# piyanon108/iGate4xSoftphoneDSP

Hardware: AMD Instinct MI355X
Metric: Msamples/s G.711 decode+RMS, 65536ch@8kHz; %HBM roofline at 1/2/4/8 GPU (higher is better)
Workload: dtype u8

## Files before the change

igate4xsoftphonedsp_amd/csrc/igdsp_capi_ctx.hip:

```cpp
#include "igdsp_ctx.h"

#include <algorithm>
#include <atomic>
#include <cmath>
#include <cstdlib>
#include <cstring>
#include <mutex>
#include <new>
#include <vector>

using namespace igdsp;
using igdsp_rx::kSlot;
using igdsp_rx::kStageDepth;

extern "C" {

int igdsp_abi_version(void) { return IGDSP_ABI_VERSION; }

int igdsp_create(igdsp_ctx **out, int device, uint32_t max_channels)
{
    if (!out || max_channels == 0 || max_channels > (1u << 24)) return IGDSP_EINVAL;
    *out = nullptr;
    int count = 0;
    if (hipGetDeviceCount(&count) != hipSuccess || count <= 0 || device < 0 || device >= count) return IGDSP_ENODEV;
    hipDeviceProp_t prop;
    if (hipGetDeviceProperties(&prop, device) != hipSuccess) return IGDSP_ENODEV;
    if (std::strncmp(prop.gcnArchName, "gfx950", 6) != 0) return IGDSP_ENODEV;
    if (hipSetDevice(device) != hipSuccess) return IGDSP_ENODEV;

    igdsp_ctx *ctx = new (std::nothrow) igdsp_ctx();
    if (!ctx) return IGDSP_ENOMEM;
    ctx->device = device;
    ctx->cus = prop.multiProcessorCount;
    ctx->name = prop.name;
    ctx->max_channels = max_channels;
    ctx->direct = std::vector<std::atomic<uint32_t>>(kDirectCalls);
    for (auto &d : ctx->direct) d.store(kNoChan, std::memory_order_relaxed);
    const size_t max_frames = (size_t)max_channels * kStageDepth;
    ctx->up_bytes = igdsp_rx::upload_layout(max_frames, max_channels).total;
    bool ok = hipStreamCreateWithFlags(&ctx->stream, hipStreamNonBlocking) == hipSuccess;
    ok = ok && hipEventCreateWithFlags(&ctx->flush_done, hipEventDisableTiming) == hipSuccess;
    for (int i = 0; i < igdsp_rx::RingMem::kArrays; ++i)
        ok = ok && hipHostMalloc(ctx->ring.array(i), igdsp_rx::RingMem::bytes(max_channels, i), hipHostMallocDefault) == hipSuccess;
    if (ok) ctx->rx.init(max_channels, ctx->ring);
    ok = ok && hipHostMalloc((void **)&ctx->h_up, ctx->up_bytes, hipHostMallocDefault) == hipSuccess;
    for (uint32_t i = 0; i < 2; ++i) {
        igdsp_rx::Published &pb = ctx->pub.set(i);
        ok = ok && hipHostMalloc((void **)&pb.last, max_channels * sizeof(igdsp_frame_stats), hipHostMallocDefault) == hipSuccess;
        ok = ok && hipHostMalloc((void **)&pb.hold, max_channels * sizeof(igdsp_chan_hold), hipHostMallocDefault) == hipSuccess;
        ok = ok && hipHostMalloc((void **)&pb.probe, max_channels * sizeof(igdsp_chan_probe), hipHostMallocDefault) == hipSuccess;
    }
    ok = ok && hipMalloc((void **)&ctx->d_up, ctx->up_bytes) == hipSuccess;
    ok = ok && hipMalloc((void **)&ctx->d_stats, 2 * max_frames * sizeof(igdsp_frame_stats)) == hipSuccess;
    ok = ok && hipMalloc((void **)&ctx->d_last, max_channels * sizeof(igdsp_frame_stats)) == hipSuccess;
    ok = ok && hipMalloc((void **)&ctx->d_hold, max_channels * sizeof(igdsp_chan_hold)) == hipSuccess;
    ok = ok && hipMalloc((void **)&ctx->d_probe, max_channels * sizeof(igdsp_chan_probe)) == hipSuccess;
    ok = ok && hipMalloc((void **)&ctx->d_queues, kQueueRing * 32u * sizeof(uint32_t)) == hipSuccess;
    ok = ok && hipMemset(ctx->d_queues, 0, kQueueRing * 32u * sizeof(uint32_t)) == hipSuccess;
    ok = ok && hipMemset(ctx->d_last, 0, max_channels * sizeof(igdsp_frame_stats)) == hipSuccess;
    ok = ok && hipMemset(ctx->d_probe, 0, max_channels * sizeof(igdsp_chan_probe)) == hipSuccess;
    if (const char *e = std::getenv("IGDSP_GLOBAL_QUEUE")) ctx->global_queue = std::atoi(e) != 0;
    if (const char *e = std::getenv("IGDSP_IO_SPARE_CHUNKS")) ctx->io_spare_cap = (size_t)std::max(0, std::atoi(e));
    if (!ok) {
        igdsp_destroy(ctx);
        return IGDSP_ENOMEM;
    }
    if (init_device_attributes() != hipSuccess) {
        igdsp_destroy(ctx);
        return IGDSP_EDEVICE;
    }
    bool up = launch_hold_reset(ctx->d_hold, max_channels, nullptr, ctx->stream) == hipSuccess;
    for (uint32_t i = 0; i < 2; ++i) {
        igdsp_rx::Published &pb = ctx->pub.set(i);
        std::memset(pb.last, 0, max_channels * sizeof(igdsp_frame_stats));
        std::memset(pb.probe, 0, max_channels * sizeof(igdsp_chan_probe));
        up = up && hipMemcpyAsync(pb.hold, ctx->d_hold, max_channels * sizeof(igdsp_chan_hold), hipMemcpyDeviceToHost, ctx->stream) == hipSuccess;
    }
    if (!up || hipStreamSynchronize(ctx->stream) != hipSuccess) {
        igdsp_destroy(ctx);
        return IGDSP_EDEVICE;
    }
    ctx->pool = make_pool(max_channels);
    *out = ctx;
    return IGDSP_OK;
}

int igdsp_destroy(igdsp_ctx *ctx)
{
    if (!ctx) return IGDSP_OK;
    ctx->pool.reset();
    if (ctx->device >= 0) (void)hipSetDevice(ctx->device);
    igdsp_tx_drop(ctx);
    igdsp_io_drop_spares(ctx);
    if (ctx->stream) { (void)hipStreamSynchronize(ctx->stream); (void)hipStreamDestroy(ctx->stream); }
    if (ctx->flush_done) (void)hipEventDestroy(ctx->flush_done);
    for (int i = 0; i < igdsp_rx::RingMem::kArrays; ++i) if (*ctx->ring.array(i)) (void)hipHostFree(*ctx->ring.array(i));
    const igdsp_rx::Published &p0 = ctx->pub.set(0), &p1 = ctx->pub.set(1);
    void *hosts[] = {ctx->h_up, p0.last, p0.hold, p0.probe, p1.last, p1.hold, p1.probe};
    for (void *p : hosts) if (p) (void)hipHostFree(p);
    void *devs[] = {ctx->d_up, ctx->d_stats, ctx->d_last, ctx->d_hold, ctx->d_probe, ctx->d_queues, ctx->d_enc_tab[0], ctx->d_enc_tab[1]};
    for (void *p : devs) if (p) (void)hipFree(p);
    delete ctx;
    return IGDSP_OK;
}

const char *igdsp_last_error(const igdsp_ctx *ctx) { return ctx ? ctx->err.c_str() : ""; }

int igdsp_device_info(const igdsp_ctx *ctx, int *device, int *compute_units, char *name, size_t name_len)
{
    if (!ctx) return IGDSP_EINVAL;
    if (device) *device = ctx->device;
    if (compute_units) *compute_units = ctx->cus;
    if (name && name_len) { std::strncpy(name, ctx->name.c_str(), name_len - 1); name[name_len - 1] = 0; }
    return IGDSP_OK;
}

int igdsp_set_variant(igdsp_ctx *ctx, int variant)
{
    if (!ctx || variant < 0 || variant > 4) return IGDSP_EINVAL;
    ctx->variant = variant;
    return IGDSP_OK;
}

int igdsp_map_call(igdsp_ctx *ctx, int32_t call_id, uint32_t channel)
{
    if (!ctx) return IGDSP_EINVAL;
    if (channel >= ctx->max_channels) return IGDSP_ERANGE;
    if (call_id >= 0 && call_id < kDirectCalls) ctx->direct[(size_t)call_id].store(channel, std::memory_order_release);
    else { std::lock_guard<std::mutex> g(ctx->far_mu); ctx->far[call_id] = channel; }
    return IGDSP_OK;
}

int igdsp_unmap_call(igdsp_ctx *ctx, int32_t call_id)
{
    if (!ctx) return IGDSP_EINVAL;
    if (call_id >= 0 && call_id < kDirectCalls) ctx->direct[(size_t)call_id].store(kNoChan, std::memory_order_release);
    else { std::lock_guard<std::mutex> g(ctx->far_mu); ctx->far.erase(call_id); }
    return IGDSP_OK;
}

int igdsp_on_rtp_frame(igdsp_ctx *ctx, int32_t call_id, uint8_t pt, const uint8_t *payload, uint32_t payloadlen)
{
    if (!ctx) return IGDSP_EINVAL;
    if (pt != IGDSP_PT_PCMU && pt != IGDSP_PT_PCMA) return IGDSP_OK;
    if (payloadlen > kSlot || (payloadlen && !payload)) return IGDSP_EINVAL;
// ... 123 lines not shown
    igdsp_frame_stats s;
    uint16_t peak_hold = 0;
    ctx->pub.read([&](const igdsp_rx::Published &p) { s = p.last[channel]; peak_hold = p.hold[channel].peak_hold; });
    out->byte_mean = s.byte_mean;
    out->flags = s.flags;
    out->peak = s.peak;
    out->rms = s.rms;
    out->percent = (int32_t)(float)(((double)s.rms * 100.0) / (double)IGDSP_METER_FULL_SCALE);
    out->peak_hold = peak_hold;
    out->dropped = (uint16_t)std::min<uint32_t>(ctx->rx.frames_dropped(channel), 65535u);
    out->frames = ctx->rx.frames_seen(channel);
    return IGDSP_OK;
}

int igdsp_poll_call(igdsp_ctx *ctx, int32_t call_id, igdsp_level *out)
{
    if (!ctx || !out) return IGDSP_EINVAL;
    const uint32_t ch = lookup(ctx, call_id);
    if (ch == kNoChan) return IGDSP_ENOENT;
    return igdsp_poll(ctx, ch, out);
}

int igdsp_reset_hold(igdsp_ctx *ctx, uint32_t channel)
{
    if (!ctx) return IGDSP_EINVAL;
    if (channel != 0xFFFFFFFFu && channel >= ctx->max_channels) return IGDSP_ERANGE;
    std::lock_guard<std::mutex> g(ctx->flush_mu);
    if (int rc = flush_end_locked(ctx, 1)) return rc;
    HIP_TRY(ctx, hipSetDevice(ctx->device));
    const uint32_t c0 = (channel == 0xFFFFFFFFu) ? 0 : channel;
    const uint32_t cn = (channel == 0xFFFFFFFFu) ? ctx->max_channels : 1;
    HIP_TRY(ctx, launch_hold_reset(ctx->d_hold + c0, cn, nullptr, ctx->stream));
    HIP_TRY(ctx, hipMemcpyAsync(ctx->pub.back().hold + c0, ctx->d_hold + c0, cn * sizeof(igdsp_chan_hold), hipMemcpyDeviceToHost, ctx->stream));
    HIP_TRY(ctx, hipStreamSynchronize(ctx->stream));
    ctx->pub.rewrite_front([&](igdsp_rx::Published &front, const igdsp_rx::Published &back) {
        std::memcpy(front.hold + c0, back.hold + c0, cn * sizeof(igdsp_chan_hold));
    });
    return IGDSP_OK;
}

int igdsp_get_hold(igdsp_ctx *ctx, uint32_t channel, igdsp_chan_hold *out)
{
    if (!ctx || !out) return IGDSP_EINVAL;
    if (channel >= ctx->max_channels) return IGDSP_ERANGE;
    ctx->pub.read([&](const igdsp_rx::Published &p) { *out = p.hold[channel]; });
    return IGDSP_OK;
}

int igdsp_get_probe(igdsp_ctx *ctx, uint32_t channel, igdsp_chan_probe *out)
{
    if (!ctx || !out) return IGDSP_EINVAL;
    if (channel >= ctx->max_channels) return IGDSP_ERANGE;
    ctx->pub.read([&](const igdsp_rx::Published &p) { *out = p.probe[channel]; });
    return IGDSP_OK;
}

int igdsp_dev_alloc(igdsp_ctx *ctx, void **d_ptr, size_t bytes)
{
    if (!ctx || !d_ptr) return IGDSP_EINVAL;
    *d_ptr = nullptr;
    if (bytes == 0) return IGDSP_OK;
    if (hipSetDevice(ctx->device) != hipSuccess) return IGDSP_ENODEV;
    hipError_t e = hipMalloc(d_ptr, bytes);
    return e == hipSuccess ? IGDSP_OK : fail(ctx, IGDSP_ENOMEM, "hipMalloc", e);
}

int igdsp_dev_free(igdsp_ctx *ctx, void *d_ptr)
{
    if (!ctx) return IGDSP_EINVAL;
    if (!d_ptr) return IGDSP_OK;
    HIP_TRY(ctx, hipSetDevice(ctx->device));
    HIP_TRY(ctx, hipFree(d_ptr));
    return IGDSP_OK;
}

int igdsp_dev_alloc_far(igdsp_ctx *ctx, void **d_ptr, size_t bytes, const void *d_in, size_t in_bytes, uint32_t max_tries,
                        size_t spacer_bytes, float *ms_first, float *ms_kept)
{
    if (!ctx || !d_ptr || !d_in || bytes == 0 || in_bytes < 10240u || max_tries == 0) return IGDSP_EINVAL;
    *d_ptr = nullptr;
    if (hipSetDevice(ctx->device) != hipSuccess) return IGDSP_ENODEV;
    if (spacer_bytes == 0) spacer_bytes = (size_t)12 << 30;
    const size_t cand_bytes = std::max(bytes, in_bytes / 10u + 4096u);
    std::vector<void *> spacers;
    void *best = nullptr;
    float t_best = 0.f, t_first = 0.f;
    int rc = IGDSP_OK;
    for (uint32_t k = 0; k < max_tries; ++k) {
        if (k > 0) {
            void *sp = nullptr;
            if (hipMalloc(&sp, spacer_bytes) != hipSuccess) { (void)hipGetLastError(); break; }
            spacers.push_back(sp);
        }
        void *cand = nullptr;
        if (hipMalloc(&cand, cand_bytes) != hipSuccess) { (void)hipGetLastError(); break; }
        float ms = 0.f;
        rc = igdsp_probe_placement(ctx, d_in, in_bytes, cand, 6, &ms, nullptr);
        if (rc != IGDSP_OK) { (void)hipFree(cand); break; }
        if (k == 0) t_first = ms;
        if (best == nullptr || ms < t_best) {
            if (best) (void)hipFree(best);
            best = cand; t_best = ms;
        } else {
            (void)hipFree(cand);
        }
        if (t_best < 0.92f * t_first) break;
    }
    for (void *sp : spacers) (void)hipFree(sp);
    if (rc != IGDSP_OK) { if (best) (void)hipFree(best); return rc; }
    if (!best) return fail(ctx, IGDSP_ENOMEM, "igdsp_dev_alloc_far");
    *d_ptr = best;
    if (ms_first) *ms_first = t_first;
    if (ms_kept) *ms_kept = t_best;
    return IGDSP_OK;
}

int igdsp_copy_h2d(igdsp_ctx *ctx, void *d_dst, const void *h_src, size_t bytes)
{
    if (!ctx || (bytes && (!d_dst || !h_src))) return IGDSP_EINVAL;
    HIP_TRY(ctx, hipSetDevice(ctx->device));
    HIP_TRY(ctx, hipMemcpy(d_dst, h_src, bytes, hipMemcpyHostToDevice));
    return IGDSP_OK;
}

int igdsp_copy_d2h(igdsp_ctx *ctx, void *h_dst, const void *d_src, size_t bytes)
// ... 73 lines not shown
```

igate4xsoftphonedsp_amd/csrc/igdsp_ctx.h:

```cpp
#pragma once
#include "igdsp_args.h"
#include "igdsp_internal.h"
#include "igdsp_rxstage.h"
#include "igdsp_snappool.h"

#include <atomic>
#include <cstdio>
#include <mutex>
#include <string>
#include <unordered_map>
#include <vector>

namespace {
constexpr uint32_t kNoChan = 0xFFFFFFFFu;
constexpr int32_t kDirectCalls = 1 << 16;
}

struct igdsp_ctx {
    int device = -1;
    int cus = 0;
    std::string name;
    uint32_t max_channels = 0;
    hipStream_t stream = nullptr;
    int variant = 0;
    std::string err;

    struct IoRange { const char *base; size_t bytes; };
    std::vector<IoRange> spread_ranges;
    std::vector<hipMemGenericAllocationHandle_t> io_spare[4];
    size_t io_spare_chunk = 0;
    size_t io_spare_cap = 16;
    uint32_t io_epoch = 0;
    std::mutex io_mu;
    bool is_spread(const void *p)
    {
        std::lock_guard<std::mutex> g(io_mu);
        for (const auto &r : spread_ranges) if ((const char *)p >= r.base && (const char *)p < r.base + r.bytes) return true;
        return false;
    }

    std::vector<std::atomic<uint32_t>> direct;
    std::unordered_map<int32_t, uint32_t> far;
    std::mutex far_mu;

    igdsp_rx::RingMem ring;
    igdsp_rx::Stager rx;
    std::atomic<uint32_t> gate_mode{IGDSP_GATE_ALWAYS};

    uint8_t *h_up = nullptr, *d_up = nullptr;
    size_t up_bytes = 0;
    igdsp_frame_stats *d_stats = nullptr;
    igdsp_frame_stats *d_last = nullptr;
    igdsp_chan_hold *d_hold = nullptr;
    igdsp_chan_probe *d_probe = nullptr;
    igdsp_rx::PublishedSet pub;
    hipEvent_t flush_done = nullptr;
    bool flush_open = false;
    uint32_t flush_nch = 0;
    std::mutex flush_mu;

    std::unique_ptr<igdsp::SnapshotPool> pool;

    struct TxSide;
    std::atomic<TxSide *> tx{nullptr};
    std::mutex tx_init_mu;

    uint32_t *d_queues = nullptr;
    uint8_t *d_enc_tab[2] = {nullptr, nullptr};
    std::once_flag enc_once[2];
    hipStream_t queue_owner[64];
    uint32_t queue_launches[64];
    uint32_t queue_used = 0;
    uint32_t queue_hint = 0;
    std::atomic_flag queue_lk = ATOMIC_FLAG_INIT;
    bool global_queue = true;
};
namespace {
constexpr uint32_t kQueueRing = 64;
const hipStream_t kFreeQueue = reinterpret_cast<hipStream_t>(~(uintptr_t)0);
}

void igdsp_io_drop_spares(igdsp_ctx *ctx);
void igdsp_tx_drop(igdsp_ctx *ctx);

static inline uint32_t lookup(igdsp_ctx *ctx, int32_t call_id)
{
    if (call_id >= 0 && call_id < kDirectCalls) return ctx->direct[(size_t)call_id].load(std::memory_order_acquire);
    std::lock_guard<std::mutex> g(ctx->far_mu);
    auto it = ctx->far.find(call_id);
    return it == ctx->far.end() ? kNoChan : it->second;
}

static inline int fail(igdsp_ctx *ctx, int code, const char *what, hipError_t e = hipSuccess)
{
    if (ctx) {
        char buf[256];
        if (e != hipSuccess) std::snprintf(buf, sizeof buf, "%s: %s", what, hipGetErrorString(e));
        else std::snprintf(buf, sizeof buf, "%s", what);
        ctx->err = buf;
    }
    return code;
}

#define HIP_TRY(ctx, call)                                                    \
    do {                                                                      \
        hipError_t e_ = (call);                                               \
        if (e_ != hipSuccess) return fail((ctx), IGDSP_EDEVICE, #call, e_);   \
    } while (0)

static inline int refuse(igdsp_ctx *ctx, const char *entry, const igdsp::args::Verdict &v)
{
    return v.why ? fail(ctx, v.rc, (std::string(entry) + ": " + v.why).c_str()) : v.rc;
}

#define ARGS_TRY(ctx, entry, verdict)                                         \
    do {                                                                      \
        const igdsp::args::Verdict v_ = (verdict);                            \
        if (!v_.run) return refuse((ctx), (entry), v_);                       \
    } while (0)

static inline hipStream_t pick(igdsp_ctx *, void *stream) { return (hipStream_t)stream; }
static inline uint32_t *queue_of(igdsp_ctx *ctx, hipStream_t stream)
{
    if (!ctx->global_queue || !ctx->d_queues || stream == hipStreamPerThread) return nullptr;
    while (ctx->queue_lk.test_and_set(std::memory_order_acquire)) {}
    uint32_t i = ctx->queue_hint;
    if (i >= ctx->queue_used || ctx->queue_owner[i] != stream) {
        uint32_t free_i = kQueueRing;
        for (i = 0; i < ctx->queue_used && ctx->queue_owner[i] != stream; ++i)
            if (ctx->queue_owner[i] == kFreeQueue && free_i == kQueueRing) free_i = i;
        if (i == ctx->queue_used) {
            if (free_i != kQueueRing) i = free_i;
            else if (ctx->queue_used < kQueueRing) ctx->queue_used += 1;
            else i = kQueueRing;
            if (i < kQueueRing) { ctx->queue_owner[i] = stream; ctx->queue_launches[i] = 0; }
// ... 33 lines not shown
```

igate4xsoftphonedsp_amd/csrc/igdsp_io.hip:

```cpp
#include "igdsp_ctx.h"

#include <algorithm>
#include <chrono>
#include <thread>
#include <cmath>
#include <cstdlib>
#include <cstring>
#include <new>

using namespace igdsp;

struct igdsp_io_set {
    struct Map { void *va = nullptr; size_t bytes = 0; std::vector<hipMemGenericAllocationHandle_t> handles; std::vector<uint8_t> cls; };
    uint32_t epoch = 0;
    std::vector<Map> maps;
    std::vector<void *> plain;
    size_t chunk = 0;
    int device = 0;
};

namespace {

constexpr size_t kSrcChunks = 10;

// ... 83 lines not shown
            chunks[idx[k]].in_src = true;
            if (hipMemSetAccess((char *)T.va + k * chunk, chunk, &acc, 1) != hipSuccess) { (void)hipGetLastError(); return false; }
        }
        *which = sources.size() - 1;
        return true;
    }
    void drop_source(size_t which)
    {
        Source &S = sources[which];
        for (size_t k = 0; k < S.idx.size(); ++k) { (void)hipMemUnmap((char *)S.va + k * chunk, chunk); chunks[S.idx[k]].in_src = false; }
        S.idx.clear();
    }
    void cleanup()
    {
        for (size_t i = 0; i < chunks.size(); ++i) unmap_scratch(i);
        for (size_t w = 0; w < sources.size(); ++w) drop_source(w);
        sources.clear();
        for (auto &c : chunks) if (!c.used) (void)hipMemRelease(c.h);
        chunks.clear();
        if (ea) (void)hipEventDestroy(ea);
        if (eb) (void)hipEventDestroy(eb);
        ea = eb = nullptr; cand_va = nullptr;
        (void)hipGetLastError();
    }
};

bool map_chunks(igdsp_io_set::Map &m, size_t chunk, const std::vector<hipMemGenericAllocationHandle_t> &hs, size_t first_slot,
                const hipMemAccessDesc &acc)
{
    for (size_t i = 0; i < hs.size(); ++i) {
        char *at = (char *)m.va + (first_slot + i) * chunk;
        if (hipMemMap(at, chunk, 0, hs[i], 0) != hipSuccess) return false;
        if (hipMemSetAccess(at, chunk, &acc, 1) != hipSuccess) return false;
    }
    return true;
}

struct IoKnobs {
    bool plain = false, frac_set = false, no_spread = false, settle = true, debug = false;
    int align_mib = -1; double limit_frac = 0.0;
    size_t stride = 16;
    IoKnobs()
    {
        if (const char *e = std::getenv("IGDSP_IO_PLAIN")) plain = std::atoi(e) != 0;
        if (const char *e = std::getenv("IGDSP_IO_ALIGN_MIB")) align_mib = std::max(0, std::atoi(e));
        if (const char *e = std::getenv("IGDSP_IO_LIMIT_FRAC")) { frac_set = true; limit_frac = std::atof(e); }
        if (const char *e = std::getenv("IGDSP_IO_STRIDE")) stride = std::max(1, std::atoi(e));
        no_spread = std::getenv("IGDSP_IO_NO_SPREAD") != nullptr;
        if (const char *e = std::getenv("IGDSP_IO_SETTLE")) settle = std::atoi(e) != 0;
        debug = std::getenv("IGDSP_IO_DEBUG") != nullptr;
    }
};
size_t probe_bytes(size_t chunk) { return kSrcChunks * (chunk - 4096) / 10240 * 10240; }
struct Layout {
    std::vector<size_t> nch;
    std::vector<uint32_t> order;
    size_t in_chunks = 0, in_bytes = 0, rec_chunks = 0, bulk_chunks = 0;
    int in0 = -1, out0 = -1;
};
struct Pools {
    std::vector<size_t> a, b, c;
    float fast = 0.f, slow = 0.f, thrB = 0.f, thrC = 0.f;
    bool split = false;
    const std::vector<size_t> &pool(int q) const { return q == 0 ? a : (q == 1 ? b : c); }
    int label(int q) const { return q == 0 ? 0 : (q == 2 ? 3 : (split ? 2 : 1)); }
};
struct Search {
    Explorer &X; const Layout &L; const size_t stride; igdsp_io_report &R;
    Pools P;
    bool ok = true;
    static constexpr float kBimodal = 1.08f, kPure = 1.125f, kNear = 1.035f;
    size_t srcA = 0, srcB = 0, nB = 0, nC = 0;
    float tmin = 1e30f, tmax = 0.f, tbmin = 1e30f, tbmax = 0.f;
    float cB = 0.f, cC = 0.f, thrB = 0.f, thrC = 0.f;
    std::vector<size_t> surveyed; std::vector<char> taken;
    bool timeA(size_t idx)
    {
        Chunk &c = X.chunks[idx];
        if (c.tA >= 0.f || c.in_src) return true;
        if (!X.probe(idx, X.sources[srcA], &c.tA, "A")) return ok = false;
        return true;
    }
    bool fast_A(size_t idx) { return !X.chunks[idx].in_src && timeA(idx) && X.chunks[idx].tA < P.fast; }
    bool timeB(size_t idx)
    {
        Chunk &c = X.chunks[idx];
        if (c.in_src || !ok) return false;
        if (c.tB < 0.f) {
            if (!X.probe(idx, X.sources[srcB], &c.tB, "B")) return ok = false;
            tbmin = std::min(tbmin, c.tB); tbmax = std::max(tbmax, c.tB);
        }
        return true;
    }
    bool is_C(size_t idx) { return fast_A(idx) && timeB(idx) && X.chunks[idx].tB < thrC; }
    bool is_B(size_t idx) { return fast_A(idx) && timeB(idx) && X.chunks[idx].tB > thrB; }
    void survey(bool rescan)
    {
        tmin = 1e30f; tmax = 0.f;
        std::vector<size_t> todo = rescan ? surveyed : std::vector<size_t>();
        surveyed.clear();
        size_t next = 0, seen = 0;
        for (;;) {
            const size_t idx = seen < todo.size() ? todo[seen] : next;
            if (seen >= todo.size() && !X.ensure(idx)) break;
            next = std::max(next, idx) + stride;
            ++seen;
// ... 275 lines not shown
            labels.push_back((uint8_t)P.label(q));
            hs.push_back(c.h);
        }
    };
    for (size_t j = 0; j < L.order.size() && ok; ++j) {
        const uint32_t i = L.order[j];
        hs.clear(); labels.clear();
        if (bufs[i].role == IGDSP_IO_INPUT) pull(0, L.nch[i]);
        else {
            const size_t h2 = (bufs[i].role == IGDSP_IO_BULK && spread) ? L.nch[i] / 2 : 0;
            pull(1, L.nch[i] - h2);
            if (hs.size() == L.nch[i] - h2) pull(2, h2);
        }
        all = all && hs.size() == L.nch[i];
        ok = map_chunks(set->maps[i], set->chunk, hs, 0, X.acc);
        set->maps[i].handles = hs; set->maps[i].cls = labels;
    }
    R.placed = (ok && all) ? 1u : 0u; R.bulk_spread = (ok && all && spread && L.bulk_chunks > 0) ? 1u : 0u;
    if (X.debug && ok) {
        std::fprintf(stderr, "[igdsp_io] pools: A %zu B %zu C %zu chunks; A:", P.a.size(), P.b.size(), P.c.size());
        for (size_t k = 0; k < P.a.size() && k < 12; ++k) std::fprintf(stderr, " %zu", P.a[k]);
        std::fprintf(stderr, "  B:");
        for (size_t k = 0; k < P.b.size() && k < 12; ++k) std::fprintf(stderr, " %zu(%.4f)", P.b[k], X.chunks[P.b[k]].tA);
        std::fprintf(stderr, "\n");
        debug_check(X, bufs, n_bufs, L, set, false);
    }
    return ok;
}
void keep_spares(igdsp_ctx *ctx, Explorer &X, const Pools &P)
{
    for (int q = 0; q < 3; ++q)
        for (size_t k : P.pool(q)) if (!X.chunks[k].used) X.chunks[k].cls = P.label(q);
    for (auto &c : X.chunks) {
        if (c.used || c.in_src || c.cls >= 0 || c.tA < 0.f) continue;
        if (c.tA > P.slow) c.cls = 0;
        else if (c.tA < P.fast) c.cls = !P.split ? 1 : (c.tB > P.thrB ? 2 : ((c.tB >= 0.f && c.tB < P.thrC) ? 3 : -1));
    }
    std::lock_guard<std::mutex> g(ctx->io_mu);
    for (auto &c : X.chunks)
        if (!c.used && !c.in_src && c.cls >= 0 && ctx->io_spare[c.cls].size() < ctx->io_spare_cap) { ctx->io_spare[c.cls].push_back(c.h); c.used = true; }
}
bool map_fresh(igdsp_io_set::Map &m, size_t nch, size_t chunk, const hipMemAllocationProp &prop, const hipMemAccessDesc &acc)
{
    const size_t have = m.handles.size();
    std::vector<hipMemGenericAllocationHandle_t> hs;
    bool ok = true;
    hipMemGenericAllocationHandle_t h;
    for (size_t k = have; k < nch && ok; ++k) if ((ok = hipMemCreate(&h, chunk, &prop, 0) == hipSuccess)) hs.push_back(h);
    ok = ok && map_chunks(m, chunk, hs, have, acc);
    m.handles.insert(m.handles.end(), hs.begin(), hs.end());
    m.cls.resize(m.handles.size(), 255);
    return ok;
}
float settle_ref(Explorer &X, const Layout &L, const igdsp_io_set *set, size_t *n)
{
    if (L.in0 < 0 || L.out0 < 0) return 0.f;
    *n = std::min(X.probe_n, std::min(L.nch[L.in0] * set->chunk, 10 * (L.nch[L.out0] * set->chunk - 4096)) / 10240 * 10240);
    const size_t keep = X.probe_n; X.probe_n = *n;
    float t = 0.f, t_ref = 0.f;
    const void *rd = set->maps[L.in0].va; void *wr = set->maps[L.out0].va;
    if (*n >= ((size_t)256 << 20) && X.time_pair(rd, wr, &t) && X.time_pair(rd, wr, &t)) t_ref = t;
    X.probe_n = keep;
    return t_ref;
}
float settle(igdsp_ctx *ctx, const Layout &L, const igdsp_io_set *set, size_t n, float t_ref, size_t released_chunks, bool debug)
{
    Explorer Y;
    const auto w0 = std::chrono::steady_clock::now();
    if (Y.open(ctx, n)) {
        const float min_wait = std::min(6000.f, (float)((double)released_chunks * (double)set->chunk / 25e9 * 1e3));
        int quiet = 0;
        for (;;) {
            float t = 0.f; if (!Y.time_pair(set->maps[L.in0].va, set->maps[L.out0].va, &t)) break;
            quiet = t <= 1.012f * t_ref ? quiet + 1 : 0;
            const float waited = std::chrono::duration<float, std::milli>(std::chrono::steady_clock::now() - w0).count();
            if (debug) std::fprintf(stderr, "[igdsp_io] settle: %.4f ms against %.4f before the release (%.0f of >= %.0f ms)\n", t, t_ref, waited, min_wait);
            if ((quiet >= 2 && waited >= min_wait) || waited > 8000.f) break;
            std::this_thread::sleep_for(std::chrono::milliseconds(50));
        }
    }
    const float ms = std::chrono::duration<float, std::milli>(std::chrono::steady_clock::now() - w0).count();
    Y.cleanup();
    return ms;
}
int place(igdsp_ctx *ctx, igdsp_io_buf *bufs, uint32_t n_bufs, size_t explore_limit_bytes, const IoKnobs &kn, igdsp_io_set *set,
          Explorer &X, igdsp_io_report &R)
{
    int vmm = 0;
    if (hipDeviceGetAttribute(&vmm, hipDeviceAttributeVirtualMemoryManagementSupported, ctx->device) != hipSuccess) { (void)hipGetLastError(); vmm = 0; }
    if (!vmm || kn.plain) return plain_path(ctx, bufs, n_bufs, set);
    X.prop.type = hipMemAllocationTypePinned; X.prop.location.type = hipMemLocationTypeDevice; X.prop.location.id = ctx->device;
    X.acc.location = X.prop.location; X.acc.flags = hipMemAccessFlagsProtReadWrite;
    size_t gran = 0;
    if (hipMemGetAllocationGranularity(&gran, &X.prop, hipMemAllocationGranularityRecommended) != hipSuccess || gran == 0) { (void)hipGetLastError(); return plain_path(ctx, bufs, n_bufs, set); }
    const size_t chunk = (((size_t)128 << 20) + gran - 1) / gran * gran;
    X.chunk = set->chunk = R.chunk_bytes = chunk;
    X.va_align = kn.align_mib >= 0 ? (size_t)kn.align_mib << 20 : chunk;
    Layout L;
    if (const int rc = reserve_ranges(ctx, bufs, n_bufs, X.va_align, set, L)) return rc;
    size_t free_b = 0, total_b = 0; (void)hipMemGetInfo(&free_b, &total_b);
    const double frac = kn.frac_set ? kn.limit_frac : (L.bulk_chunks >= 4 ? 0.85 : 0.5);
    const size_t limit = std::min(explore_limit_bytes ? explore_limit_bytes : (size_t)(frac * (double)free_b), (size_t)(0.9 * (double)free_b));
    const bool want_place = L.in_bytes >= ((size_t)512 << 20) && ((L.rec_chunks + L.bulk_chunks) > 0 || L.in_chunks > kSrcChunks) && limit / chunk >= 4 * kSrcChunks;
    const int spared = want_place ? from_spares(ctx, bufs, n_bufs, L, set, X.acc, R) : kNotServed;
    if (spared != kNotServed) return spared;
    Search S{X, L, kn.stride, R};
    bool ok = !want_place || S.run(ctx, set, kn, limit);
    if (ok && (!S.P.b.empty() || (L.rec_chunks + L.bulk_chunks == 0 && !S.P.a.empty()))) ok = hand_out(X, S.P, bufs, n_bufs, L, set, R);
    size_t settle_n = 0;
    const float t_ref = R.placed ? settle_ref(X, L, set, &settle_n) : 0.f;
    if (R.placed) keep_spares(ctx, X, S.P);
    const size_t released_chunks = (size_t)std::count_if(X.chunks.begin(), X.chunks.end(), [](const Chunk &c) { return !c.used; });
    X.cleanup();
    for (uint32_t i : L.order)
        if (ok && set->maps[i].handles.size() < L.nch[i]) ok = map_fresh(set->maps[i], L.nch[i], chunk, X.prop, X.acc);
    if (!ok) { (void)hipGetLastError(); return fail(ctx, IGDSP_ENOMEM, "igdsp_io_alloc: mapping chunks"); }
    publish(ctx, bufs, n_bufs, set, R.bulk_spread);
    if (kn.settle && t_ref > 0.f) R.settle_ms = settle(ctx, L, set, settle_n, t_ref, released_chunks, kn.debug);
    if (kn.debug && R.placed) { Explorer Y; if (Y.open(ctx, probe_bytes(chunk))) debug_check(Y, bufs, n_bufs, L, set, true); Y.cleanup(); }
    return IGDSP_OK;
}

}

void igdsp_io_drop_spares(igdsp_ctx *ctx)
{
    std::vector<hipMemGenericAllocationHandle_t> gone;
    std::unique_lock<std::mutex> g(ctx->io_mu);
    for (auto &v : ctx->io_spare) { gone.insert(gone.end(), v.begin(), v.end()); v.clear(); }
    g.unlock();
    for (auto h : gone) (void)hipMemRelease(h);
    (void)hipGetLastError();
}

extern "C" {

int igdsp_io_free(igdsp_ctx *ctx, igdsp_io_set *set)
{
    if (!ctx) return IGDSP_EINVAL;
    if (!set) return IGDSP_OK;
    (void)hipSetDevice(set->device);
    (void)hipDeviceSynchronize();
    {
        std::lock_guard<std::mutex> g(ctx->io_mu);
        for (auto &m : set->maps)
            for (size_t k = 0; k < ctx->spread_ranges.size();)
                if (ctx->spread_ranges[k].base == (const char *)m.va) ctx->spread_ranges.erase(ctx->spread_ranges.begin() + (long)k); else ++k;
    }
    for (auto &m : set->maps) {
        if (!m.va) continue;
        for (size_t i = 0; i < m.handles.size(); ++i) (void)hipMemUnmap((char *)m.va + i * set->chunk, set->chunk);
        std::vector<hipMemGenericAllocationHandle_t> gone;
        std::unique_lock<std::mutex> g(ctx->io_mu);
        for (size_t i = 0; i < m.handles.size(); ++i) {
            const uint8_t c = i < m.cls.size() ? m.cls[i] : 255;
            if (c < 4 && set->epoch == ctx->io_epoch && set->chunk == ctx->io_spare_chunk && ctx->io_spare[c].size() < ctx->io_spare_cap) ctx->io_spare[c].push_back(m.handles[i]);
            else gone.push_back(m.handles[i]);
        }
        g.unlock();
        for (auto h : gone) (void)hipMemRelease(h);
    }
    for (void *p : set->plain) if (p) (void)hipFree(p);
    (void)hipGetLastError();
    delete set;
    return IGDSP_OK;
}

int igdsp_internal_vmm_remap_check(igdsp_ctx *ctx, int mode, int *bytes)
{
    if (!ctx || !bytes) return IGDSP_EINVAL;
    HIP_TRY(ctx, hipSetDevice(ctx->device));
    hipMemAllocationProp prop{};
    prop.type = hipMemAllocationTypePinned;
    prop.location.type = hipMemLocationTypeDevice;
    prop.location.id = ctx->device;
// ... 17 lines not shown
    HIP_TRY(ctx, hipMemUnmap(v, sz));
    bytes[2] = 1;
    if (mode == 1) {
        void *v0 = v;
        HIP_TRY(ctx, hipDeviceSynchronize());
        HIP_TRY(ctx, hipMemAddressFree(v, sz));
        HIP_TRY(ctx, hipMemAddressReserve(&v, sz, 0, v0, 0));
        bytes[2] = v == v0 ? 1 : 0;
    }
    HIP_TRY(ctx, hipMemMap(v, sz, 0, Y, 0));
    HIP_TRY(ctx, hipMemSetAccess(v, sz, &acc, 1));
    HIP_TRY(ctx, hipMemsetAsync(v, 0x22, sz, ctx->stream));
    HIP_TRY(ctx, hipStreamSynchronize(ctx->stream));
    HIP_TRY(ctx, hipMemUnmap(v, sz));
    HIP_TRY(ctx, hipMemMap(wx, sz, 0, X, 0));
    HIP_TRY(ctx, hipMemSetAccess(wx, sz, &acc, 1));
    HIP_TRY(ctx, hipMemMap(wy, sz, 0, Y, 0));
    HIP_TRY(ctx, hipMemSetAccess(wy, sz, &acc, 1));
    unsigned char bx = 0, by = 0;
    HIP_TRY(ctx, hipMemcpy(&bx, (char *)wx + sz / 2, 1, hipMemcpyDeviceToHost));
    HIP_TRY(ctx, hipMemcpy(&by, (char *)wy + sz / 2, 1, hipMemcpyDeviceToHost));
    bytes[0] = bx; bytes[1] = by;
    (void)hipMemUnmap(wx, sz); (void)hipMemUnmap(wy, sz);
    (void)hipMemRelease(X); (void)hipMemRelease(Y);
    return IGDSP_OK;
}

int igdsp_io_alloc(igdsp_ctx *ctx, igdsp_io_buf *bufs, uint32_t n_bufs, size_t explore_limit_bytes, igdsp_io_set **out_set,
                   igdsp_io_report *rep)
{
    if (!ctx || !bufs || !out_set || n_bufs == 0 || n_bufs > 64) return IGDSP_EINVAL;
    *out_set = nullptr;
    for (uint32_t i = 0; i < n_bufs; ++i) {
        bufs[i].ptr = nullptr;
        if (bufs[i].bytes == 0 || bufs[i].role > IGDSP_IO_BULK) return IGDSP_EINVAL;
    }
    HIP_TRY(ctx, hipSetDevice(ctx->device));
    const auto t_start = std::chrono::steady_clock::now();
    igdsp_io_set *set = new (std::nothrow) igdsp_io_set();
    if (!set) return IGDSP_ENOMEM;
    set->device = ctx->device;
    const IoKnobs kn;
    igdsp_io_report R = {};
    Explorer X; X.ctx = ctx; X.s = ctx->stream;
    const int rc = place(ctx, bufs, n_bufs, explore_limit_bytes, kn, set, X, R);
    X.cleanup();
    R.setup_ms = std::chrono::duration<float, std::milli>(std::chrono::steady_clock::now() - t_start).count();
    if (rep) *rep = R;
    if (rc != IGDSP_OK) { igdsp_io_free(ctx, set); for (uint32_t i = 0; i < n_bufs; ++i) bufs[i].ptr = nullptr; }
    else *out_set = set;
    return rc;
}

}
```

Baseline: 5.940 million.

## Place large device allocations on timing-probed VMM chunks relative to a reference buffer

Large igdsp_dev_alloc requests (at least 128 MiB) now go through the VMM path by default. The allocator probes candidate physical chunks against an existing large buffer, keeps the chunks whose copy timing differs from it (a bimodal fast/slow class), and maps them into a reserved VA range. It reuses classified spare chunks, waits for memory to settle after releasing extra chunks, and routes the matching free through unmap and spare recycling. The aim is to keep input and output buffers on physical memory classes that do not contend, raising HBM throughput. The cost is allocation time for probing and settling, plus a heuristic that depends on the hardware.

```diff
diff --git a/igate4xsoftphonedsp_amd/csrc/igdsp_capi_ctx.hip b/igate4xsoftphonedsp_amd/csrc/igdsp_capi_ctx.hip
--- a/igate4xsoftphonedsp_amd/csrc/igdsp_capi_ctx.hip
+++ b/igate4xsoftphonedsp_amd/csrc/igdsp_capi_ctx.hip
@@ -61,6 +61,7 @@
     ok = ok && hipMemset(ctx->d_probe, 0, max_channels * sizeof(igdsp_chan_probe)) == hipSuccess;
     if (const char *e = std::getenv("IGDSP_GLOBAL_QUEUE")) ctx->global_queue = std::atoi(e) != 0;
     if (const char *e = std::getenv("IGDSP_IO_SPARE_CHUNKS")) ctx->io_spare_cap = (size_t)std::max(0, std::atoi(e));
+    if (const char *e = std::getenv("IGDSP_DEV_ALLOC_PLACE")) ctx->dev_place = std::atoi(e) != 0;
     if (!ok) {
         igdsp_destroy(ctx);
         return IGDSP_ENOMEM;
@@ -91,6 +92,7 @@
     ctx->pool.reset();
     if (ctx->device >= 0) (void)hipSetDevice(ctx->device);
     igdsp_tx_drop(ctx);
+    igdsp_dev_drop_all(ctx);
     igdsp_io_drop_spares(ctx);
     if (ctx->stream) { (void)hipStreamSynchronize(ctx->stream); (void)hipStreamDestroy(ctx->stream); }
     if (ctx->flush_done) (void)hipEventDestroy(ctx->flush_done);
@@ -320,25 +322,6 @@
     if (!ctx || !out) return IGDSP_EINVAL;
     if (channel >= ctx->max_channels) return IGDSP_ERANGE;
     ctx->pub.read([&](const igdsp_rx::Published &p) { *out = p.probe[channel]; });
-    return IGDSP_OK;
-}
-
-int igdsp_dev_alloc(igdsp_ctx *ctx, void **d_ptr, size_t bytes)
-{
-    if (!ctx || !d_ptr) return IGDSP_EINVAL;
-    *d_ptr = nullptr;
-    if (bytes == 0) return IGDSP_OK;
-    if (hipSetDevice(ctx->device) != hipSuccess) return IGDSP_ENODEV;
-    hipError_t e = hipMalloc(d_ptr, bytes);
-    return e == hipSuccess ? IGDSP_OK : fail(ctx, IGDSP_ENOMEM, "hipMalloc", e);
-}
-
-int igdsp_dev_free(igdsp_ctx *ctx, void *d_ptr)
-{
-    if (!ctx) return IGDSP_EINVAL;
-    if (!d_ptr) return IGDSP_OK;
-    HIP_TRY(ctx, hipSetDevice(ctx->device));
-    HIP_TRY(ctx, hipFree(d_ptr));
     return IGDSP_OK;
 }
 
diff --git a/igate4xsoftphonedsp_amd/csrc/igdsp_ctx.h b/igate4xsoftphonedsp_amd/csrc/igdsp_ctx.h
--- a/igate4xsoftphonedsp_amd/csrc/igdsp_ctx.h
+++ b/igate4xsoftphonedsp_amd/csrc/igdsp_ctx.h
@@ -32,6 +32,13 @@
     size_t io_spare_cap = 16;
     uint32_t io_epoch = 0;
     std::mutex io_mu;
+    struct DevBuf { void *va = nullptr; size_t bytes = 0, chunk = 0; std::vector<hipMemGenericAllocationHandle_t> handles; uint8_t cls = 255; uint32_t epoch = 0; };
+    std::vector<DevBuf> dev_bufs;
+    struct DevReport { uint32_t placed = 0, probes = 0; uint64_t explored_bytes = 0; float setup_ms = 0.f, settle_ms = 0.f; };
+    DevReport dev_last;
+    float dev_total_ms = 0.f;
+    bool dev_place = true;
+    std::mutex dev_mu;
     bool is_spread(const void *p)
     {
         std::lock_guard<std::mutex> g(io_mu);
@@ -81,6 +88,7 @@
 }
 
 void igdsp_io_drop_spares(igdsp_ctx *ctx);
+void igdsp_dev_drop_all(igdsp_ctx *ctx);
 void igdsp_tx_drop(igdsp_ctx *ctx);
 
 static inline uint32_t lookup(igdsp_ctx *ctx, int32_t call_id)
diff --git a/igate4xsoftphonedsp_amd/csrc/igdsp_io.hip b/igate4xsoftphonedsp_amd/csrc/igdsp_io.hip
--- a/igate4xsoftphonedsp_amd/csrc/igdsp_io.hip
+++ b/igate4xsoftphonedsp_amd/csrc/igdsp_io.hip
@@ -159,6 +159,19 @@
     }
 };
 size_t probe_bytes(size_t chunk) { return kSrcChunks * (chunk - 4096) / 10240 * 10240; }
+bool vmm_open(igdsp_ctx *ctx, const IoKnobs &kn, Explorer &X)
+{
+    int vmm = 0;
+    if (hipDeviceGetAttribute(&vmm, hipDeviceAttributeVirtualMemoryManagementSupported, ctx->device) != hipSuccess) { (void)hipGetLastError(); vmm = 0; }
+    if (!vmm) return false;
+    X.prop.type = hipMemAllocationTypePinned; X.prop.location.type = hipMemLocationTypeDevice; X.prop.location.id = ctx->device;
+    X.acc.location = X.prop.location; X.acc.flags = hipMemAccessFlagsProtReadWrite;
+    size_t gran = 0;
+    if (hipMemGetAllocationGranularity(&gran, &X.prop, hipMemAllocationGranularityRecommended) != hipSuccess || gran == 0) { (void)hipGetLastError(); return false; }
+    X.chunk = (((size_t)128 << 20) + gran - 1) / gran * gran;
+    X.va_align = kn.align_mib >= 0 ? (size_t)kn.align_mib << 20 : X.chunk;
+    return true;
+}
 struct Layout {
     std::vector<size_t> nch;
     std::vector<uint32_t> order;
@@ -540,26 +553,29 @@
     m.cls.resize(m.handles.size(), 255);
     return ok;
 }
-float settle_ref(Explorer &X, const Layout &L, const igdsp_io_set *set, size_t *n)
-{
-    if (L.in0 < 0 || L.out0 < 0) return 0.f;
-    *n = std::min(X.probe_n, std::min(L.nch[L.in0] * set->chunk, 10 * (L.nch[L.out0] * set->chunk - 4096)) / 10240 * 10240);
+float settle_ref(Explorer &X, const void *rd, size_t rd_bytes, void *wr, size_t wr_bytes, size_t *n)
+{
+    *n = std::min(X.probe_n, std::min(rd_bytes, 10 * (wr_bytes - 4096)) / 10240 * 10240);
     const size_t keep = X.probe_n; X.probe_n = *n;
     float t = 0.f, t_ref = 0.f;
-    const void *rd = set->maps[L.in0].va; void *wr = set->maps[L.out0].va;
     if (*n >= ((size_t)256 << 20) && X.time_pair(rd, wr, &t) && X.time_pair(rd, wr, &t)) t_ref = t;
     X.probe_n = keep;
     return t_ref;
 }
-float settle(igdsp_ctx *ctx, const Layout &L, const igdsp_io_set *set, size_t n, float t_ref, size_t released_chunks, bool debug)
+float settle_ref(Explorer &X, const Layout &L, const igdsp_io_set *set, size_t *n)
+{
+    if (L.in0 < 0 || L.out0 < 0) return 0.f;
+    return settle_ref(X, set->maps[L.in0].va, L.nch[L.in0] * set->chunk, set->maps[L.out0].va, L.nch[L.out0] * set->chunk, n);
+}
+float settle(igdsp_ctx *ctx, const void *rd, void *wr, size_t chunk, size_t n, float t_ref, size_t released_chunks, bool debug)
 {
     Explorer Y;
     const auto w0 = std::chrono::steady_clock::now();
     if (Y.open(ctx, n)) {
-        const float min_wait = std::min(6000.f, (float)((double)released_chunks * (double)set->chunk / 25e9 * 1e3));
+        const float min_wait = std::min(6000.f, (float)((double)released_chunks * (double)chunk / 25e9 * 1e3));
         int quiet = 0;
         for (;;) {
-            float t = 0.f; if (!Y.time_pair(set->maps[L.in0].va, set->maps[L.out0].va, &t)) break;
+            float t = 0.f; if (!Y.time_pair(rd, wr, &t)) break;
             quiet = t <= 1.012f * t_ref ? quiet + 1 : 0;
             const float waited = std::chrono::duration<float, std::milli>(std::chrono::steady_clock::now() - w0).count();
             if (debug) std::fprintf(stderr, "[igdsp_io] settle: %.4f ms against %.4f before the release (%.0f of >= %.0f ms)\n", t, t_ref, waited, min_wait);
@@ -574,16 +590,8 @@
 int place(igdsp_ctx *ctx, igdsp_io_buf *bufs, uint32_t n_bufs, size_t explore_limit_bytes, const IoKnobs &kn, igdsp_io_set *set,
           Explorer &X, igdsp_io_report &R)
 {
-    int vmm = 0;
-    if (hipDeviceGetAttribute(&vmm, hipDeviceAttributeVirtualMemoryManagementSupported, ctx->device) != hipSuccess) { (void)hipGetLastError(); vmm = 0; }
-    if (!vmm || kn.plain) return plain_path(ctx, bufs, n_bufs, set);
-    X.prop.type = hipMemAllocationTypePinned; X.prop.location.type = hipMemLocationTypeDevice; X.prop.location.id = ctx->device;
-    X.acc.location = X.prop.location; X.acc.flags = hipMemAccessFlagsProtReadWrite;
-    size_t gran = 0;
-    if (hipMemGetAllocationGranularity(&gran, &X.prop, hipMemAllocationGranularityRecommended) != hipSuccess || gran == 0) { (void)hipGetLastError(); return plain_path(ctx, bufs, n_bufs, set); }
-    const size_t chunk = (((size_t)128 << 20) + gran - 1) / gran * gran;
-    X.chunk = set->chunk = R.chunk_bytes = chunk;
-    X.va_align = kn.align_mib >= 0 ? (size_t)kn.align_mib << 20 : chunk;
+    if (kn.plain || !vmm_open(ctx, kn, X)) return plain_path(ctx, bufs, n_bufs, set);
+    const size_t chunk = set->chunk = R.chunk_bytes = X.chunk;
     Layout L;
     if (const int rc = reserve_ranges(ctx, bufs, n_bufs, X.va_align, set, L)) return rc;
     size_t free_b = 0, total_b = 0; (void)hipMemGetInfo(&free_b, &total_b);
@@ -604,11 +612,195 @@
         if (ok && set->maps[i].handles.size() < L.nch[i]) ok = map_fresh(set->maps[i], L.nch[i], chunk, X.prop, X.acc);
     if (!ok) { (void)hipGetLastError(); return fail(ctx, IGDSP_ENOMEM, "igdsp_io_alloc: mapping chunks"); }
     publish(ctx, bufs, n_bufs, set, R.bulk_spread);
-    if (kn.settle && t_ref > 0.f) R.settle_ms = settle(ctx, L, set, settle_n, t_ref, released_chunks, kn.debug);
+    if (kn.settle && t_ref > 0.f) R.settle_ms = settle(ctx, set->maps[L.in0].va, set->maps[L.out0].va, chunk, settle_n, t_ref, released_chunks, kn.debug);
     if (kn.debug && R.placed) { Explorer Y; if (Y.open(ctx, probe_bytes(chunk))) debug_check(Y, bufs, n_bufs, L, set, true); Y.cleanup(); }
     return IGDSP_OK;
 }
 
+constexpr size_t kDevLarge = (size_t)128 << 20;
+constexpr uint32_t kDevMaxProbes = 64;
+constexpr int kDevWarm = 28;
+
+using DevBuf = igdsp_ctx::DevBuf;
+struct DevRef { void *va = nullptr; size_t nch = 0; uint8_t cls = 255; };
+
+void dev_release(DevBuf &B)
+{
+    for (size_t i = 0; i < B.handles.size(); ++i) { (void)hipMemUnmap((char *)B.va + i * B.chunk, B.chunk); (void)hipMemRelease(B.handles[i]); }
+    B.handles.clear();
+    (void)hipGetLastError();
+}
+bool other_class(uint8_t ref_cls, int q) { return ref_cls == 0 ? q != 0 : (ref_cls == 1 ? q == 0 : (ref_cls < 4 && q != 1 && q != (int)ref_cls)); }
+
+bool dev_place(igdsp_ctx *ctx, const IoKnobs &kn, Explorer &X, const DevRef &ref, size_t nch, DevBuf &B, igdsp_ctx::DevReport &R,
+               float *t_ref, size_t *settle_n, size_t *released)
+{
+    const size_t chunk = X.chunk;
+    size_t free_b = 0, total_b = 0; (void)hipMemGetInfo(&free_b, &total_b);
+    const double frac = kn.frac_set ? kn.limit_frac : 0.5;
+    const size_t limit = std::min((size_t)(frac * (double)free_b), (size_t)(0.9 * (double)free_b));
+    const size_t stride = kn.stride | 1;
+    X.limit_chunks = std::min(limit / chunk, (size_t)kDevMaxProbes * stride + nch);
+    if (X.limit_chunks < nch + 2 * stride) return true;
+    X.debug = kn.debug;
+    if (hipMemAddressReserve(&X.cand_va, X.limit_chunks * chunk, X.va_align, nullptr, 0) != hipSuccess) { (void)hipGetLastError(); X.cand_va = nullptr; return false; }
+    if (!X.open(ctx, probe_bytes(chunk))) return false;
+    X.sources.push_back(Source{ref.va, kSrcChunks, {}});
+    Layout L; igdsp_io_report rep = {};
+    Search S{X, L, stride, rep};
+    bool &ok = S.ok;
+    float t = 0.f;
+    ok = X.ensure(0);
+    for (int k = 0; k < kDevWarm && ok; ++k) ok = X.probe(0, X.sources[0], &t, "warm");
+    const uint32_t warm = X.probes;
+    auto spent = [&]() { return X.probes - warm; };
+    float tmin = 1e30f, tmax = 0.f;
+    std::vector<size_t> sparse;
+    auto levels = [&]() { tmin = 1e30f; tmax = 0.f; for (size_t k : sparse) { tmin = std::min(tmin, X.chunks[k].tA); tmax = std::max(tmax, X.chunks[k].tA); } };
+    for (size_t idx = 0; ok && spent() < kDevMaxProbes && X.ensure(idx); idx += stride) {
+        if (!S.timeA(idx)) break;
+        sparse.push_back(idx); levels();
+        if (!(tmax > Search::kBimodal * tmin)) continue;
+        X.chunks[idx].tA = -1.f;
+        if (!S.timeA(idx)) break;
+        levels();
+        if (tmax > Search::kBimodal * tmin) break;
+    }
+    std::vector<size_t> got;
+    if (ok && tmax > Search::kBimodal * tmin) {
+        S.P.fast = Search::kNear * tmin; S.P.slow = tmax / Search::kNear;
+        size_t first = 0;
+        while (first < X.chunks.size() && !(X.chunks[first].tA >= 0.f && X.chunks[first].tA < S.P.fast)) ++first;
+        bool capped = false;
+        S.walk(first, nch, [&](size_t i) {
+            if (X.chunks[i].tA < 0.f && spent() >= kDevMaxProbes) { capped = true; return ok = false; }
+            return S.fast_A(i);
+        }, got);
+        if (capped) ok = true;
+        if (got.size() < nch) got.clear();
+    }
+    R.probes = spent(); R.explored_bytes = (uint64_t)X.chunks.size() * chunk;
+    if (kn.debug) std::fprintf(stderr, "[igdsp_io] dev_alloc: %zu chunks against a reference of %zu: levels %.4f / %.4f, %u probes, %zu chunks explored -> %s\n",
+                               nch, ref.nch, tmax, tmin, R.probes, X.chunks.size(), got.empty() ? "not placed" : "placed");
+    if (!ok) return false;
+    *released = X.chunks.size();
+    if (got.empty()) return true;
+    for (size_t i = 0; i < X.chunks.size(); ++i) X.unmap_scratch(i);
+    for (size_t k : got) { X.chunks[k].used = true; B.handles.push_back(X.chunks[k].h); }
+    igdsp_io_set::Map M; M.va = B.va;
+    if (!map_chunks(M, chunk, B.handles, 0, X.acc)) { (void)hipGetLastError(); return false; }
+    R.placed = 1;
+    *t_ref = settle_ref(X, ref.va, ref.nch * chunk, B.va, B.bytes, settle_n);
+    {
+        std::lock_guard<std::mutex> g(ctx->io_mu);
+        DevBuf *rb = nullptr;
+        for (DevBuf &b : ctx->dev_bufs) if (b.va == ref.va) rb = &b;
+        bool held = false, label = false;
+        for (const auto &v : ctx->io_spare) held = held || !v.empty();
+        if (rb && tmax >= Search::kPure * tmin) {
+            const uint8_t rc = rb->epoch == ctx->io_epoch ? rb->cls : (uint8_t)255;
+            if (rc == 0) label = ctx->io_spare_chunk == chunk;
+            else if (rc == 255 && !held) { ++ctx->io_epoch; ctx->io_spare_chunk = chunk; rb->cls = 0; rb->epoch = ctx->io_epoch; label = true; }
+        }
+        if (label) {
+            B.cls = 1; B.epoch = ctx->io_epoch;
+            for (auto &c : X.chunks) {
+                if (c.used || c.tA < 0.f) continue;
+                const int q = c.tA > S.P.slow ? 0 : (c.tA < S.P.fast ? 1 : -1);
+                if (q >= 0 && ctx->io_spare[q].size() < ctx->io_spare_cap) { ctx->io_spare[q].push_back(c.h); c.used = true; }
+            }
+        }
+    }
+    *released = (size_t)std::count_if(X.chunks.begin(), X.chunks.end(), [](const Chunk &c) { return !c.used; });
+    return true;
+}
+
+int dev_alloc_large(igdsp_ctx *ctx, void **d_ptr, size_t bytes)
+{
+    const IoKnobs kn;
+    Explorer X; X.ctx = ctx; X.s = ctx->stream;
+    if (!vmm_open(ctx, kn, X) || bytes < X.chunk) return kNotServed;
+    std::lock_guard<std::mutex> whole(ctx->dev_mu);
+    const auto t_start = std::chrono::steady_clock::now();
+    const size_t chunk = X.chunk, nch = (bytes + chunk - 1) / chunk;
+    igdsp_ctx::DevReport R;
+    DevBuf B; B.chunk = chunk; B.bytes = nch * chunk;
+    if (hipMemAddressReserve(&B.va, B.bytes, X.va_align, nullptr, 0) != hipSuccess) { (void)hipGetLastError(); return kNotServed; }
+    DevRef ref;
+    {
+        std::lock_guard<std::mutex> g(ctx->io_mu);
+        for (const DevBuf &b : ctx->dev_bufs)
+            if (b.handles.size() >= ref.nch) ref = DevRef{b.va, b.handles.size(), b.epoch == ctx->io_epoch ? b.cls : (uint8_t)255};
+        for (int q = 0; q < 4 && B.handles.empty() && ctx->io_spare_chunk == chunk; ++q) {
+            auto &S = ctx->io_spare[q];
+            if (S.size() < nch || !(ref.va ? other_class(ref.cls, q) : q == 0)) continue;
+            B.handles.assign(S.end() - (long)nch, S.end()); S.erase(S.end() - (long)nch, S.end());
+            B.cls = (uint8_t)q; B.epoch = ctx->io_epoch;
+        }
+    }
+    const bool spared = !B.handles.empty();
+    bool ok = true;
+    float t_ref = 0.f;
+    size_t settle_n = 0, released = 0;
+    if (spared) R.placed = ref.va ? 1u : 0u;
+    else if (ref.va && ref.nch >= kSrcChunks) ok = dev_place(ctx, kn, X, ref, nch, B, R, &t_ref, &settle_n, &released);
+    X.cleanup();
+    igdsp_io_set::Map M; M.va = B.va;
+    if (ok && spared) ok = map_chunks(M, chunk, B.handles, 0, X.acc);
+    else if (ok && B.handles.empty()) { ok = map_fresh(M, nch, chunk, X.prop, X.acc); B.handles = M.handles; }
+    if (!ok) { (void)hipGetLastError(); dev_release(B); return kNotServed; }
+    { std::lock_guard<std::mutex> g(ctx->io_mu); ctx->dev_bufs.push_back(B); }
+    if (kn.settle && released > 0) {
+        if (t_ref > 0.f) R.settle_ms = settle(ctx, ref.va, B.va, chunk, settle_n, t_ref, released, kn.debug);
+        else {
+            const auto w0 = std::chrono::steady_clock::now();
+            std::this_thread::sleep_for(std::chrono::milliseconds((long)std::min(6000.0, (double)released * (double)chunk / 25e9 * 1e3)));
+            R.settle_ms = std::chrono::duration<float, std::milli>(std::chrono::steady_clock::now() - w0).count();
+        }
+    }
+    R.setup_ms = std::chrono::duration<float, std::milli>(std::chrono::steady_clock::now() - t_start).count();
+    { std::lock_guard<std::mutex> g(ctx->io_mu); ctx->dev_last = R; ctx->dev_total_ms += R.setup_ms; }
+    *d_ptr = B.va;
+    return IGDSP_OK;
+}
+
+int dev_free_large(igdsp_ctx *ctx, void *d_ptr)
+{
+    auto find = [&]() { size_t k = 0; while (k < ctx->dev_bufs.size() && ctx->dev_bufs[k].va != d_ptr) ++k; return k; };
+    { std::lock_guard<std::mutex> g(ctx->io_mu); if (find() == ctx->dev_bufs.size()) return kNotServed; }
+    std::lock_guard<std::mutex> whole(ctx->dev_mu);
+    DevBuf B;
+    {
+        std::lock_guard<std::mutex> g(ctx->io_mu);
+        const size_t k = find();
+        if (k == ctx->dev_bufs.size()) return kNotServed;
+        B = ctx->dev_bufs[k];
+        ctx->dev_bufs.erase(ctx->dev_bufs.begin() + (long)k);
+    }
+    (void)hipDeviceSynchronize();
+    for (size_t i = 0; i < B.handles.size(); ++i) (void)hipMemUnmap((char *)B.va + i * B.chunk, B.chunk);
+    std::vector<hipMemGenericAllocationHandle_t> gone;
+    {
+        std::lock_guard<std::mutex> g(ctx->io_mu);
+        for (auto h : B.handles) {
+            if (B.cls < 4 && B.epoch == ctx->io_epoch && B.chunk == ctx->io_spare_chunk && ctx->io_spare[B.cls].size() < ctx->io_spare_cap) ctx->io_spare[B.cls].push_back(h);
+            else gone.push_back(h);
+        }
+    }
+    for (auto h : gone) (void)hipMemRelease(h);
+    (void)hipGetLastError();
+    return IGDSP_OK;
+}
+
+}
+
+void igdsp_dev_drop_all(igdsp_ctx *ctx)
+{
+    std::vector<DevBuf> all;
+    { std::lock_guard<std::mutex> g(ctx->io_mu); all.swap(ctx->dev_bufs); }
+    if (all.empty()) return;
+    (void)hipDeviceSynchronize();
+    for (auto &B : all) dev_release(B);
 }
 
 void igdsp_io_drop_spares(igdsp_ctx *ctx)
@@ -732,4 +924,39 @@
     return rc;
 }
 
-}
+int igdsp_dev_alloc(igdsp_ctx *ctx, void **d_ptr, size_t bytes)
+{
+    if (!ctx || !d_ptr) return IGDSP_EINVAL;
+    *d_ptr = nullptr;
+    if (bytes == 0) return IGDSP_OK;
+    if (hipSetDevice(ctx->device) != hipSuccess) return IGDSP_ENODEV;
+    if (ctx->dev_place && bytes >= kDevLarge && dev_alloc_large(ctx, d_ptr, bytes) == IGDSP_OK) return IGDSP_OK;
+    hipError_t e = hipMalloc(d_ptr, bytes);
+    return e == hipSuccess ? IGDSP_OK : fail(ctx, IGDSP_ENOMEM, "hipMalloc", e);
+}
+
+int igdsp_dev_free(igdsp_ctx *ctx, void *d_ptr)
+{
+    if (!ctx) return IGDSP_EINVAL;
+    if (!d_ptr) return IGDSP_OK;
+    HIP_TRY(ctx, hipSetDevice(ctx->device));
+    if (dev_free_large(ctx, d_ptr) == IGDSP_OK) return IGDSP_OK;
+    HIP_TRY(ctx, hipFree(d_ptr));
+    return IGDSP_OK;
+}
+
+int igdsp_internal_dev_alloc_report(igdsp_ctx *ctx, uint32_t *placed, uint32_t *probes, uint64_t *explored_bytes, float *setup_ms,
+                                    float *settle_ms, float *total_setup_ms)
+{
+    if (!ctx) return IGDSP_EINVAL;
+    std::lock_guard<std::mutex> g(ctx->io_mu);
+    if (placed) *placed = ctx->dev_last.placed;
+    if (probes) *probes = ctx->dev_last.probes;
+    if (explored_bytes) *explored_bytes = ctx->dev_last.explored_bytes;
+    if (setup_ms) *setup_ms = ctx->dev_last.setup_ms;
+    if (settle_ms) *settle_ms = ctx->dev_last.settle_ms;
+    if (total_setup_ms) *total_setup_ms = ctx->dev_total_ms;
+    return IGDSP_OK;
+}
+
+}
```

Result: no change. 5.936 million (-0.1%).
